# guoyihonggyh/MOBODY-Model-Based-Off-Dynamics-Offline-Reinforcement-Learning

Hardware: AMD Instinct MI355X
Metric: transitions/sec (minibatch rows through train(), refresh amortised at 1/5000) + grad-steps/sec (higher is better)
Workload: dtype f16x2

## Files before the change

### mobody-model-based-off-dynamics-offline-reinforcement-learning_amd/csrc/layers.h

```cpp
#pragma once
#include <stdint.h>
#include <stdlib.h>

#include <type_traits>

#include "../../include/mobody_hip.h"
#include "gather.h"
#include "tile.h"

namespace mobody {

template <int ACT, int MT, class Extra, class Between>
__device__ __forceinline__ void wide_layer(float* Xs, const float* __restrict__ W, const float* __restrict__ b, int Kp,
                                           WideRing& ring, Extra&& extra, Between&& between, uint32_t* mask = nullptr,
                                           bool full = false, int mask_groups = 1 << 30) {
  const float bias0 = b[64 * wave_col() + (lane_id() & 31)], bias1 = b[64 * wave_col() + 32 + (lane_id() & 31)];
  f32x16 acc[MT][2];
  wide_zero<MT>(acc);
  wide_gemm<MT>(Xs, W, Kp, acc, ring);
  if (Kp == HID) TR(3);
  between();
  lds_barrier();
  if (full) {
    wide_foreach<MT>(acc, [&](int row, int col, float v) {
// ... 82 lines not shown
  const unsigned short* w2_planes;
  long long planes_ms;
  float* save_d1;
  float* save_d2;
  unsigned short* save_h1p;
  long long h1p_ms;
  long long h1p_plane;
  int* save_e1;
  int out_mode;
  const float* resid;
  int resid_ld;
  float max_action;
};

constexpr long long DYN_PLANE_MEMBER = 3LL * HID * HID;
__host__ __device__ inline long long dyn_planes_off(int layer, int member) { return ((long long)layer * NENS + member) * DYN_PLANE_MEMBER; }

inline Mlp3FwdArgs fwd_net(const float* blob, const MobodyMlpLayout& L, long long rows) {
  Mlp3FwdArgs a{};
  a.w1 = blob + L.w1; a.b1 = blob + L.b1; a.w2 = blob + L.w2; a.b2 = blob + L.b2; a.w3 = blob + L.w3; a.b3 = blob + L.b3;
  a.sw1 = a.sb1 = a.sw2 = a.sb2 = a.sw3 = a.sb3 = L.member_floats;
  a.Kp1 = L.Kp1; a.Np3 = L.Np3; a.nout = L.out_dim; a.rows = rows;
  return a;
}
inline void fwd_set_planes(Mlp3FwdArgs& a, const float* blob_T, const MobodyMlpLayout& L) {
  a.w2_planes = reinterpret_cast<const unsigned short*>(blob_T + L.w2p);
  a.planes_ms = 2 * L.t_member_floats;
}
inline Mlp3FwdArgs fwd_reward_head(const float* dyn_blob, const MobodyDynLayout& L, const float* dyn_planes, long long rows) {
  Mlp3FwdArgs a{};
  const MobodyLayer &l1 = L.layer[MOBODY_DL_RW1], &l2 = L.layer[MOBODY_DL_RW2], &l3 = L.layer[MOBODY_DL_RW3];
  a.w1 = dyn_blob + l1.w_off; a.b1 = dyn_blob + l1.b_off; a.sw1 = (long long)l1.Kp * l1.Np; a.sb1 = l1.Np;
  a.w2 = dyn_blob + l2.w_off; a.b2 = dyn_blob + l2.b_off; a.sw2 = (long long)l2.Kp * l2.Np; a.sb2 = l2.Np;
  a.w3 = dyn_blob + l3.w_off; a.b3 = dyn_blob + l3.b_off; a.sw3 = (long long)l3.Kp * l3.Np; a.sb3 = l3.Np;
  a.Kp1 = l1.Kp; a.Np3 = l3.Np; a.nout = 1; a.rows = rows;
  if (dyn_planes != nullptr) {
    a.w2_planes = reinterpret_cast<const unsigned short*>(dyn_planes) + dyn_planes_off(2, 0);
    a.planes_ms = DYN_PLANE_MEMBER;
  }
  return a;
}
inline void fwd_set_src(Mlp3FwdArgs& a, int k, const float* src, int ld, int n, long long ms = 0) {
  a.src[k] = src; a.ld[k] = ld; a.n[k] = n; a.src_ms[k] = ms;
}
inline void fwd_set_out(Mlp3FwdArgs& a, float* out, int out_mode, float max_action, const float* resid = nullptr, int resid_ld = 0) {
  a.out = out; a.out_mstride = a.rows * a.nout; a.out_ld = a.nout;
  a.out_mode = out_mode; a.max_action = max_action; a.resid = resid; a.resid_ld = resid_ld;
}
inline void fwd_set_saves(Mlp3FwdArgs& a, float* x, long long x_ms, float* h1, int* e1, float* h2, uint32_t* m1 = nullptr,
                          uint32_t* m2 = nullptr, float* d1 = nullptr, float* d2 = nullptr) {
  if (e1 != nullptr && h1 != nullptr) {
    const long long r32 = (a.rows + 31) & ~31LL;
    a.save_h1p = reinterpret_cast<unsigned short*>(h1); a.h1p_plane = r32 * HID; a.h1p_ms = 2 * r32 * HID; a.save_e1 = e1;
    h1 = nullptr;
  }
  a.save_x = x; a.x_ms = x_ms; a.save_h1 = h1; a.save_h2 = h2; a.mask1 = m1; a.mask2 = m2; a.save_d1 = d1; a.save_d2 = d2;
}

struct FwdGather {
  GatherArgs g;
  int off[2], n[2];
};
inline void fwd_set_gather(FwdGather& fg, int k, const Mlp3FwdArgs& a, int off) {
  fg.off[k] = off; fg.n[k] = a.n[0] + a.n[1] + a.n[2];
}
constexpr int FWD_GATHER_NQ = 2;

template <class F>
inline int dispatch_out_width(int Np3, F&& f) {
  return Np3 == 16 ? f(std::integral_constant<int, 1>{}) : Np3 == 32 ? f(std::integral_constant<int, 2>{})
                                                                     : f(std::integral_constant<int, 0>{});
}

int launch_mlp3_forward(const Mlp3FwdArgs& a, int members_a, const Mlp3FwdArgs& b, int members_b, int act, int prec, hipStream_t st);
inline int launch_mlp3_forward(const Mlp3FwdArgs& a, int members, int act, int prec, hipStream_t st) {
  return launch_mlp3_forward(a, members, Mlp3FwdArgs{}, 0, act, prec, st);
}

int launch_mlp3_forward_gather(const Mlp3FwdArgs& a, int members_a, const Mlp3FwdArgs& b, int members_b, const FwdGather& fg,
                               int prec, hipStream_t st);
int launch_mlp3_fwd_bf_gather(const Mlp3FwdArgs& a, int members_a, const Mlp3FwdArgs& b, int members_b, const FwdGather& fg,
                              int prec, hipStream_t st);

constexpr int MLP_TILE_ROWS = 32;
constexpr int MLP_MT = MLP_TILE_ROWS / 32;

__device__ __forceinline__ int fwd_load_sources(const Mlp3FwdArgs& a, int m, float* Xs, long long row0, int rows_here) {
  int c0 = 0;
#pragma unroll
  for (int k = 0; k < 3; ++k) {
    if (a.n[k] > 0) {
      tile_load(Xs, c0, a.src[k] + m * a.src_ms[k] + row0 * a.ld[k], a.ld[k], a.n[k], 0, rows_here, MLP_TILE_ROWS);
      c0 += a.n[k];
    }
  }
  return c0;
}

template <int NQ>
__device__ __forceinline__ void fwd_gather_rows(const FwdGather& fg, bool second, float* Xs, long long row0, int rows_here) {
  const GatherArgs& g = fg.g;
  const int lane = threadIdx.x & 15, grp = threadIdx.x >> 4;
  const long long N = g.start[g.nbuf];
  const float* mine = nullptr;
  if (lane < 2) {
    const long long r = min(row0 + 16 * lane + grp, N - 1);
    int k;
    const long long src = gather_src(g, r, k);
    mine = g.bufs[k].state + src * g.bufs[k].pitch;
  }
  const int off = second ? fg.off[1] : fg.off[0], n = second ? fg.n[1] : fg.n[0];
  const int q0 = off >> 2, q1 = (off + n + (second ? 2 : 0) + 3) >> 2;
  v4f v[2][NQ];
#pragma unroll
  for (int p = 0; p < 2; ++p) {
    const gather_ptr_t rp = gather_group_row(mine, p);
#pragma unroll
    for (int j = 0; j < NQ; ++j) v[p][j] = rp[min(q0 + lane + 16 * j, q1 - 1)];
  }
#pragma unroll
  for (int p = 0; p < 2; ++p) {
    const int r = 16 * p + grp;
    const bool ok = r < rows_here;
#pragma unroll
    for (int j = 0; j < NQ; ++j) {
      const int q = q0 + lane + 16 * j;
      if (q >= q1) continue;
#pragma unroll
      for (int e = 0; e < 4; ++e) {
        const int c = 4 * q + e - off;
        if (c >= 0 && c < n) Xs[r * LDX + c] = ok ? v[p][j][e] : 0.f;
        if (second && ok && c == n) g.reward[row0 + r] = v[p][j][e];
        if (second && ok && c == n + 1) g.not_done[row0 + r] = v[p][j][e];
      }
    }
  }
}

__device__ __forceinline__ int fwd_gather_tile(const FwdGather& fg, bool second, float* Xs, long long row0, int rows_here) {
  if (blockIdx.x == 0 && blockIdx.y == 0 && threadIdx.x == 0)
    for (int k = 0; k < fg.g.nbump; ++k) fg.g.bump[k][0] += 1;
  const int off = second ? fg.off[1] : fg.off[0], n = second ? fg.n[1] : fg.n[0];
  if (((off + n + (second ? 2 : 0) + 3) >> 2) - (off >> 2) <= 16) fwd_gather_rows<1>(fg, second, Xs, row0, rows_here);
  else fwd_gather_rows<FWD_GATHER_NQ>(fg, second, Xs, row0, rows_here);
  return n;
}

__device__ __forceinline__ void fwd_gather_save(const FwdGather& fg, bool second, int m, const float* Xs, long long row0, int rows_here) {
  const GatherArgs& g = fg.g;
  auto put = [&](float* out, int col0, int n) {
    const uint32_t magic = div_magic(n);
    for (int e = threadIdx.x; e < rows_here * n; e += NTHREADS) {
      const int r = fast_div(e, magic, n);
      out[row0 * n + e] = Xs[r * LDX + col0 + (e - r * n)];
    }
  };
  if (second) {
    put(g.next_state, 0, g.S);
  } else if (m == 0) {
    put(g.state, 0, g.S);
    put(g.action, g.S, g.A);
  }
}

__device__ __forceinline__ void fwd_save_x(const Mlp3FwdArgs& a, int m, const float* Xs, long long row0, int rows_here) {
  if (a.save_x != nullptr && (m == 0 || a.x_ms != 0)) {
    const int c = threadIdx.x & 31, r0 = threadIdx.x >> 5;
    float* sx = a.save_x + m * a.x_ms;
    for (int col = c; col < a.Kp1; col += 32)
      for (int r = r0; r < rows_here; r += NTHREADS >> 5) sx[(row0 + r) * a.Kp1 + col] = Xs[r * LDX + col];
  }
}

struct FwdTileOut { float *h1, *h2; uint32_t *mask1, *mask2; float* out; };
__device__ __forceinline__ FwdTileOut fwd_tile_out(const Mlp3FwdArgs& a, int m, long long row0) {
  FwdTileOut t;
  t.h1 = a.save_h1 ? a.save_h1 + ((long long)m * a.rows + row0) * HID : nullptr;
  t.h2 = a.save_h2 ? a.save_h2 + ((long long)m * a.rows + row0) * HID : nullptr;
  const long long mtile = ((long long)m * ((a.rows + 31) / 32) + row0 / 32) * HID;
  t.mask1 = a.mask1 ? a.mask1 + mtile : nullptr;
  t.mask2 = a.mask2 ? a.mask2 + mtile : nullptr;
  t.out = a.out + m * a.out_mstride + row0 * a.out_ld;
  return t;
}

__device__ __forceinline__ void fwd_emit(const Mlp3FwdArgs& a, float* out, long long row0, int rows_here, int row, int col,
                                         float v, float bias) {
  if (row < rows_here && col < a.nout) {
    float y = v + bias;
    if (a.out_mode == 1) y = a.max_action * tanhf(y);
    if (a.resid != nullptr) y += a.resid[(row0 + row) * a.resid_ld + col];
    out[row * a.out_ld + col] = y;
  }
}

}
```

### mobody-model-based-off-dynamics-offline-reinforcement-learning_amd/csrc/mlp_fwd.hip

```cpp
#include <stdlib.h>

#include "common.h"
#include "layers.h"

namespace mobody {

constexpr int TB = MLP_TILE_ROWS;

template <int ACT, int NT>
__device__ __forceinline__ void mlp3_fwd_tail(const Mlp3FwdArgs& a, int m, float* Xs, WideRing& ring, float* h2,
                                              uint32_t* mask2, float* out, long long row0, int rows_here) {
  const float* w3 = a.w3 + m * a.sw3;
  const float* b3 = a.b3 + m * a.sb3;
  const bool full = rows_here == TB;
  auto save_h2 = [=](auto guarded, int row, int col, float y) {
    if (h2 != nullptr && (!decltype(guarded)::value || row < rows_here)) h2[row * HID + col] = y;
  };
  auto emit = [&](int row, int col, float v, float bias) { fwd_emit(a, out, row0, rows_here, row, col, v, bias); };
  if constexpr (NT > 0) {
    NarrowRegs<NT> br;
    const int mycol = threadIdx.x % (16 * NT);
    float bias;
    wide_layer<ACT, MLP_MT>(Xs, a.w2 + m * a.sw2, a.b2 + m * a.sb2, HID, ring, save_h2, [&] {
      narrow_prefetch<NT>(w3, 16 * NT, br);
// ... 82 lines not shown
  if (!once) {
    int rc = allow_big_lds(k_mlp3_fwd2<ACT_RELU, NT>, 160 * 1024);
    if (rc) return rc;
    once = true;
  }
  const long long rows = a.rows > b.rows ? a.rows : b.rows;
  dim3 grid((unsigned)cdiv(rows, TB), (unsigned)(members_a + members_b));
  ProfScope prof(PROF_MLP_FWD, stream);
  hipLaunchKernelGGL((k_mlp3_fwd2<ACT_RELU, NT>), grid, dim3(NTHREADS), lds, stream, a, b, members_a);
  MB_LAUNCH_OK("k_mlp3_fwd2");
  return 0;
}

static int launch_fwd2_gather(const Mlp3FwdArgs& a, int members_a, const Mlp3FwdArgs& b, int members_b, const FwdGather& fg, hipStream_t stream) {
  size_t lds = (size_t)TB * LDX * sizeof(float);
  static bool once = false;
  if (!once) {
    int rc = allow_big_lds(k_mlp3_fwd2_gather<1>, 160 * 1024);
    if (rc) return rc;
    once = true;
  }
  dim3 grid((unsigned)cdiv(a.rows, TB), (unsigned)(members_a + members_b));
  ProfScope prof(PROF_MLP_FWD, stream);
  hipLaunchKernelGGL(k_mlp3_fwd2_gather<1>, grid, dim3(NTHREADS), lds, stream, a, b, members_a, fg);
  MB_LAUNCH_OK("k_mlp3_fwd2_gather");
  return 0;
}

static int launch_fwd_pair(const Mlp3FwdArgs& a, int members_a, const Mlp3FwdArgs& b, int members_b, hipStream_t stream) {
  return dispatch_out_width(a.Np3, [&](auto nt) { return launch_fwd2_t<decltype(nt)::value>(a, members_a, b, members_b, stream); });
}

template <int ACT>
static int launch_fwd_act(const Mlp3FwdArgs& a, int members, hipStream_t stream) {
  return dispatch_out_width(a.Np3, [&](auto nt) { return launch_fwd_t<ACT, decltype(nt)::value>(a, members, stream); });
}

static int launch_mlp3_fwd(const Mlp3FwdArgs& a, int members, int act, hipStream_t stream) {
  return act == ACT_SWISH ? launch_fwd_act<ACT_SWISH>(a, members, stream) : launch_fwd_act<ACT_RELU>(a, members, stream);
}

int launch_mlp3_fwd_bf(const Mlp3FwdArgs& a, int members_a, const Mlp3FwdArgs& b, int members_b, int act, int prec, hipStream_t st);
int launch_fwd_train(const Mlp3FwdArgs& a, int members, hipStream_t st);

static bool nets_share_launch(const Mlp3FwdArgs& a, const Mlp3FwdArgs& b, int act, int prec) {
  if (act != ACT_RELU) return false;
  return a.Np3 == b.Np3 || (prec == PREC_F16X2 && ((a.Np3 == 16 && b.Np3 == 32) || (a.Np3 == 32 && b.Np3 == 16)));
}

int launch_mlp3_forward(const Mlp3FwdArgs& a, int members_a, const Mlp3FwdArgs& b, int members_b, int act, int prec, hipStream_t st) {
  auto one = [&](const Mlp3FwdArgs& x, int members) {
    if (prec != PREC_F32) return launch_mlp3_fwd_bf(x, members, Mlp3FwdArgs{}, 0, act, prec, st);
    return x.save_d1 != nullptr ? launch_fwd_train(x, members, st) : launch_mlp3_fwd(x, members, act, st);
  };
  const bool has_a = members_a > 0 && a.rows > 0, has_b = members_b > 0 && b.rows > 0;
  if (!has_a || !has_b) return has_a ? one(a, members_a) : has_b ? one(b, members_b) : 0;
  if (!nets_share_launch(a, b, act, prec)) {
    int rc = one(a, members_a);
    return rc ? rc : one(b, members_b);
  }
  return prec == PREC_F32 ? launch_fwd_pair(a, members_a, b, members_b, st) : launch_mlp3_fwd_bf(a, members_a, b, members_b, act, prec, st);
}

int launch_mlp3_forward_gather(const Mlp3FwdArgs& a, int members_a, const Mlp3FwdArgs& b, int members_b, const FwdGather& fg,
                               int prec, hipStream_t st) {
  const GatherArgs& g = fg.g;
  const long long N = g.start[g.nbuf];
  if (N <= 0 || members_a <= 0 || members_b <= 0) return fail(MOBODY_E_ARG, "launch_mlp3_forward_gather: needs both nets and a non-empty minibatch");
  if (a.rows != N || b.rows != N) return fail(MOBODY_E_ARG, "launch_mlp3_forward_gather: the nets run on %lld / %lld rows, the minibatch has %lld", a.rows, b.rows, N);
  for (int k = 0; k < g.nbuf; ++k)
    if (!g.packed[k] && g.start[k + 1] > g.start[k]) return fail(MOBODY_E_ARG, "launch_mlp3_forward_gather: source %d is not a packed ring", k);
  if (fg.off[0] != 0 || fg.n[0] != g.S + g.A || fg.off[1] != g.S + g.A || fg.n[1] != g.S)
    return fail(MOBODY_E_ARG, "launch_mlp3_forward_gather: net a reads state | action, net b next_state");
  auto chunks = [](int off, int n) { return ((off + n + 3) >> 2) - (off >> 2); };
  const bool built = a.Np3 == 16 && (b.Np3 == 16 || (prec == PREC_F16X2 && b.Np3 == 32)) && nets_share_launch(a, b, ACT_RELU, prec) &&
                     chunks(fg.off[0], fg.n[0]) <= 16 * FWD_GATHER_NQ && chunks(fg.off[1], fg.n[1] + 2) <= 16 * FWD_GATHER_NQ;
  if (!built) {
    int rc = launch_gather(g, N, st);
    return rc ? rc : launch_mlp3_forward(a, members_a, b, members_b, ACT_RELU, prec, st);
  }
  return prec == PREC_F32 ? launch_fwd2_gather(a, members_a, b, members_b, fg, st) : launch_mlp3_fwd_bf_gather(a, members_a, b, members_b, fg, prec, st);
}

}

using namespace mobody;

extern "C" int mobody_mlp3_forward(const float* blob, const float* blob_T, int precision, int in_dim, int out_dim,
                                   int members, const float* src0, int n0, const float* src1, int n1, int64_t rows,
                                   int out_mode, float max_action, float* out, float* save_x, float* save_h1,
                                   float* save_h2, void* stream) {
  MobodyMlpLayout L;
  int rc = mobody_mlp_layout(in_dim, out_dim, members, &L);
  if (rc) return rc;
  MB_REQUIRE(rows >= 0, "mobody_mlp3_forward: rows < 0");
  if (rows == 0) return 0;
  MB_REQUIRE(blob && src0 && out, "mobody_mlp3_forward: null pointer");
  MB_REQUIRE(n0 + n1 == in_dim && n0 > 0 && n1 >= 0 && (n1 == 0 || src1), "mobody_mlp3_forward: n0+n1=%d != in_dim=%d", n0 + n1, in_dim);
  rc = check_precision("mobody_mlp3_forward", precision, blob_T != nullptr);
  if (rc) return rc;
  Mlp3FwdArgs a = fwd_net(blob, L, rows);
  fwd_set_src(a, 0, src0, n0, n0);
  fwd_set_src(a, 1, src1, n1, n1);
  fwd_set_out(a, out, out_mode, max_action);
  fwd_set_saves(a, save_x, 0, save_h1, nullptr, save_h2);
  if (precision != PREC_F32) fwd_set_planes(a, blob_T, L);
  return launch_mlp3_forward(a, members, ACT_RELU, precision, as_stream(stream));
}
```

### mobody-model-based-off-dynamics-offline-reinforcement-learning_amd/csrc/mlp_fwd_bf.hip

```cpp
#include <stdlib.h>

#include "common.h"
#include "layers_bf.h"

namespace mobody {

constexpr int TB = MLP_TILE_ROWS, MT = MLP_MT;
constexpr int FWD_L1_RING = 3;
constexpr int FWD_F16_WAVES = 4;

template <int ACT, int PM, int NT, bool DS = false, bool GATHER = false>
__device__ __forceinline__ void mlp3_fwd_bf_tile(const Mlp3FwdArgs& a, int m, float* Xs, const FwdGather* fg = nullptr, bool second = false) {
  char* Ps = reinterpret_cast<char*>(Xs);
  float* scr = reinterpret_cast<float*>(Ps + split_scr_offset<PM, TB>());
  const long long row0 = (long long)blockIdx.x * TB;
  const int rows_here = (int)min((long long)TB, a.rows - row0);
  const bool full = rows_here == TB;
  const float* w1 = a.w1 + m * a.sw1;
  const s16x8* w2b = reinterpret_cast<const s16x8*>(a.w2_planes + m * a.planes_ms);
  const float* w3 = a.w3 + m * a.sw3;
  const float* b3 = a.b3 + m * a.sb3;
  TR(0);
  WideRingT<FWD_L1_RING> ring;
  wide_prefetch(w1, a.Kp1, ring);
  int c0;
  if constexpr (GATHER) {
    c0 = fwd_gather_tile(*fg, second, Xs, row0, rows_here);
  } else if (a.n[0] <= 32 && a.n[1] <= 32 && a.n[2] == 0) {
    tile_load2<TB>(Xs, a.src[0] + m * a.src_ms[0] + row0 * a.ld[0], a.ld[0], a.n[0],
                   a.n[1] > 0 ? a.src[1] + m * a.src_ms[1] + row0 * a.ld[1] : nullptr, a.ld[1], a.n[1], rows_here);
    c0 = a.n[0] + a.n[1];
  } else {
    c0 = fwd_load_sources(a, m, Xs, row0, rows_here);
  }
  tile_zero_cols(Xs, c0, a.Kp1, TB);
  lds_barrier();
  TR(1);
  fwd_save_x(a, m, Xs, row0, rows_here);
  if constexpr (GATHER) fwd_gather_save(*fg, second, m, Xs, row0, rows_here);
  const FwdTileOut t = fwd_tile_out(a, m, row0);
  float* d1 = DS ? a.save_d1 + ((long long)m * a.rows + row0) * HID : nullptr;
  float* d2 = DS ? a.save_d2 + ((long long)m * a.rows + row0) * HID : nullptr;
  const int mg = (rows_here + 31) / 32;
  BfRing<PM> bring;
  PlaneSave gs{nullptr, 0, nullptr};
  if (a.save_h1p != nullptr) {
    gs.base = reinterpret_cast<short*>(a.save_h1p) + m * a.h1p_ms + (row0 / 8) * (HID * 8);
    gs.plane_stride = a.h1p_plane;
    gs.e_out = a.save_e1 + (long long)m * cdiv(a.rows, 32) + row0 / 32;
  }
  const int e1 = wide_layer_to_planes<ACT, MT, PM, TB, DS>(Xs, Ps, scr, w1, a.b1 + m * a.sb1, a.Kp1, ring,
                                                           [&] { bf_prefetch<PM>(w2b, bring); }, t.mask1, full, mg, rows_here, t.h1, gs, d1);
  TR(2);
  auto emit = [&](int row, int col, float v, float bias) { fwd_emit(a, t.out, row0, rows_here, row, col, v, bias); };
  if constexpr (NT > 0) {
    NarrowRegs<NT> br;
    const int mycol = threadIdx.x % (16 * NT);
    float bias;
    bf_layer<ACT, MT, PM, TB, DS>(Xs, Ps, e1, w2b, a.b2 + m * a.sb2, bring, [&] {
      narrow_prefetch<NT>(w3, 16 * NT, br);
      bias = b3[mycol < a.nout ? mycol : 0];
    }, t.mask2, mg, rows_here, t.h2, d2);
    TR(4);
    narrow_run<TB / 16, NT>(Xs, br, [&](int row, int col, float v) { emit(row, col, v, bias); });
  } else {
    bf_layer<ACT, MT, PM, TB, DS>(Xs, Ps, e1, w2b, a.b2 + m * a.sb2, bring, [] {}, t.mask2, mg, rows_here, t.h2, d2);
    narrow_layer(Xs, w3, HID, a.Np3, [&](int row, int col, float v) { emit(row, col, v, b3[col < a.nout ? col : 0]); }, TB);
  }
  TR(5);
}

template <int ACT, int PM, int NT, bool DS = false, int NT2 = NT>
__global__ __launch_bounds__(NTHREADS, (PM == 4 && !DS) ? FWD_F16_WAVES : 2) void k_mlp3_fwd_bf(Mlp3FwdArgs a, Mlp3FwdArgs b, int members_a) {
  extern __shared__ __attribute__((aligned(16))) float Xs[];
  const bool second = (int)blockIdx.y >= members_a;
  const Mlp3FwdArgs s = second ? b : a;
  if ((long long)blockIdx.x * TB >= s.rows) return;
  if constexpr (NT2 == NT) {
    mlp3_fwd_bf_tile<ACT, PM, NT, DS>(s, second ? (int)blockIdx.y - members_a : (int)blockIdx.y, Xs);
  } else {
    if (second) mlp3_fwd_bf_tile<ACT, PM, NT2, DS>(s, (int)blockIdx.y - members_a, Xs);
    else mlp3_fwd_bf_tile<ACT, PM, NT, DS>(s, (int)blockIdx.y, Xs);
  }
}

template <int PM, int NT, int NT2 = NT>
__global__ __launch_bounds__(NTHREADS, PM == 4 ? FWD_F16_WAVES : 2) void k_mlp3_fwd_bf_gather(Mlp3FwdArgs a, Mlp3FwdArgs b, int members_a, FwdGather fg) {
  extern __shared__ __attribute__((aligned(16))) float Xs[];
  const bool second = (int)blockIdx.y >= members_a;
  const Mlp3FwdArgs s = second ? b : a;
  if ((long long)blockIdx.x * TB >= s.rows) return;
  if constexpr (NT2 == NT) {
    mlp3_fwd_bf_tile<ACT_RELU, PM, NT, false, true>(s, second ? (int)blockIdx.y - members_a : (int)blockIdx.y, Xs, &fg, second);
  } else {
    if (second) mlp3_fwd_bf_tile<ACT_RELU, PM, NT2, false, true>(s, (int)blockIdx.y - members_a, Xs, &fg, true);
    else mlp3_fwd_bf_tile<ACT_RELU, PM, NT, false, true>(s, (int)blockIdx.y, Xs, &fg, false);
  }
}

template <int PM, int NT, int NT2 = NT>
static int launch_bf_gather_t(const Mlp3FwdArgs& a, int members_a, const Mlp3FwdArgs& b, int members_b, const FwdGather& fg, hipStream_t st) {
  constexpr size_t lds = split_lds_bytes<PM, TB>();
  static bool once = false;
  if (!once) {
    int rc = allow_big_lds(k_mlp3_fwd_bf_gather<PM, NT, NT2>, 160 * 1024);
    if (rc) return rc;
    once = true;
  }
  ProfScope prof(PROF_MLP_FWD, st);
  hipLaunchKernelGGL((k_mlp3_fwd_bf_gather<PM, NT, NT2>), dim3((unsigned)cdiv(a.rows, TB), (unsigned)(members_a + members_b)),
                     dim3(NTHREADS), lds, st, a, b, members_a, fg);
  MB_LAUNCH_OK("k_mlp3_fwd_bf_gather");
  return 0;
}

int launch_mlp3_fwd_bf_gather(const Mlp3FwdArgs& a, int members_a, const Mlp3FwdArgs& b, int members_b, const FwdGather& fg,
                              int prec, hipStream_t st) {
  if (prec == PREC_F16X2 && b.Np3 == 32) return launch_bf_gather_t<4, 1, 2>(a, members_a, b, members_b, fg, st);
  switch (prec) {
    case PREC_BF16: return launch_bf_gather_t<1, 1>(a, members_a, b, members_b, fg, st);
    case PREC_BF16X2: return launch_bf_gather_t<2, 1>(a, members_a, b, members_b, fg, st);
    case PREC_BF16X3: return launch_bf_gather_t<3, 1>(a, members_a, b, members_b, fg, st);
    default: return launch_bf_gather_t<4, 1>(a, members_a, b, members_b, fg, st);
  }
}

template <int ACT, int PM, int NT, bool DS = false, int NT2 = NT>
static int launch_bf_t(const Mlp3FwdArgs& a, int members_a, const Mlp3FwdArgs& b, int members_b, hipStream_t st) {
  constexpr size_t lds = split_lds_bytes<PM, TB>();
  static bool once = false;
  if (!once) {
    int rc = allow_big_lds(k_mlp3_fwd_bf<ACT, PM, NT, DS, NT2>, 160 * 1024);
    if (rc) return rc;
    once = true;
  }
  const long long rows = a.rows > b.rows ? a.rows : b.rows;
  ProfScope prof(PROF_MLP_FWD, st);
  hipLaunchKernelGGL((k_mlp3_fwd_bf<ACT, PM, NT, DS, NT2>), dim3((unsigned)cdiv(rows, TB), (unsigned)(members_a + members_b)),
                     dim3(NTHREADS), lds, st, a, b, members_a);
  MB_LAUNCH_OK("k_mlp3_fwd_bf");
  return 0;
}

template <int ACT, int PM>
static int launch_bf_nt(const Mlp3FwdArgs& a, int ma, const Mlp3FwdArgs& b, int mb, hipStream_t st) {
  if constexpr (PM == 4 && ACT == ACT_RELU) {
    if (mb > 0 && a.Np3 != b.Np3)
      return a.Np3 == 16 ? launch_bf_t<ACT, PM, 1, false, 2>(a, ma, b, mb, st) : launch_bf_t<ACT, PM, 2, false, 1>(a, ma, b, mb, st);
  }
  return dispatch_out_width(a.Np3, [&](auto nt) { return launch_bf_t<ACT, PM, decltype(nt)::value>(a, ma, b, mb, st); });
}

int launch_mlp3_fwd_bf(const Mlp3FwdArgs& a, int members_a, const Mlp3FwdArgs& b, int members_b, int act, int prec, hipStream_t st) {
// ... 13 lines not shown
```

### mobody-model-based-off-dynamics-offline-reinforcement-learning_amd/csrc/train.hip

```cpp
#include <math.h>

#include "common.h"
#include "layers.h"
#include "train.h"

namespace mobody {

struct TrainWs {
  uint32_t *mq1, *mq2, *ma1, *ma2;
  int *eh1q, *eh1a, *edz2;
  float *pin;
  float *pi, *qt, *q, *qb, *xq, *h1q, *h2q, *xa, *h1a, *h2a, *dz3q, *dz2, *dz1, *dz3a, *dxa, *bcw, *dbp, *slabs, *lossp;
  float *bc;
  int *tickets;
  long long total;
  int nsplit_q, nsplit_a, ntiles;
  MobodyMlpLayout Lq, La;
};

static int carve(const MobodyTrainDims& d, float* base, TrainWs& w) {
  int rc = mobody_mlp_layout(d.S + d.A, 1, 2, &w.Lq);
  if (rc) return rc;
  rc = mobody_mlp_layout(d.S, d.A, 1, &w.La);
  if (rc) return rc;
// ... 158 lines not shown
                            long long rows, float* out, int out_mode, float max_action, float* sx, float* sh1,
                            float* sh2, uint32_t* m1 = nullptr, uint32_t* m2 = nullptr, const float* blob_T = nullptr,
                            int* e1 = nullptr) {
  Mlp3FwdArgs a = fwd_net(blob, L, rows);
  if (blob_T != nullptr) fwd_set_planes(a, blob_T, L);
  fwd_set_src(a, 0, s0, n0, n0);
  fwd_set_src(a, 1, s1, n1, s1 ? n1 : 0);
  fwd_set_out(a, out, out_mode, max_action);
  fwd_set_saves(a, sx, 0, sh1, e1, sh2, m1, m2);
  return a;
}

static int weight_grads(const MobodyMlpLayout& L, const float* x, const float* h1, const float* h2, const int* e_h1, const float* dz3,
                        long long rows, const TrainWs& w, float* grad, const LossFinal& loss, const AdamTarget& adam, int prec,
                        hipStream_t st) {
  const bool actor = L.members == 1;
  Mlp3WgradArgs g = wgrad_net(L, rows, actor ? w.nsplit_a : w.nsplit_q);
  wgrad_set_saves(g, x, 0, h1, h2, e_h1);
  wgrad_set_grads(g, dz3, w.dz2, w.dz1, w.dbp, w.ntiles, w.edz2);
  wgrad_set_scratch(g, w.slabs, w.bc + (actor ? 2 : 0));
  wgrad_set_result(g, grad, loss, adam, prec);
  return mlp3_weight_grads(g, st);
}

static Mlp3BwdArgs bwd_args(const MobodyMlpLayout& L, const float* blob_T, const float* dz3, const float* h1,
                            const float* h2, long long rows, float* dz2, float* dz1, float* dbp,
                            const uint32_t* m1 = nullptr, const uint32_t* m2 = nullptr, int prec = PREC_F32, int* e2 = nullptr) {
  Mlp3BwdArgs b = bwd_net(L, blob_T, rows);
  bwd_set_planes(b, L, prec);
  bwd_set_acts(b, h1, h2, m1, m2, 0);
  bwd_set_grads(b, dz3, dz2, dz1, dbp, prec == PREC_F16X2 ? e2 : nullptr);
  return b;
}

}

using namespace mobody;

extern "C" int64_t mobody_train_workspace(const MobodyTrainDims* d) {
  if (check_dims(d, "mobody_train_workspace")) return -1;
  TrainWs w;
  if (carve(*d, nullptr, w)) return -1;
  return w.total;
}

static int critic_impl(const MobodyCritic& a, const FwdGather* gather, void* stream) {
  const char* who = "mobody_critic";
  const MobodyTrainDims* d = &a.d;
  const MobodyHyper* h = &a.h;
  const bool fused = a.m != nullptr;
  int rc = check_dims(d, who);
  if (rc) return rc;
  MB_REQUIRE(a.q_blob && a.q_blob_T && a.state && a.action && a.reward && a.not_done && a.loss_out && a.workspace, "%s: null pointer", who);
  MB_REQUIRE(a.q_next || (a.actor_blob && a.qtarg_blob && a.next_state), "%s: need q_next or actor/target/next_state", who);
  rc = check_precision(who, h->precision, a.q_next != nullptr || (a.actor_blob_T && a.qtarg_blob_T));
  if (rc) return rc;
  if (fused) {
    MB_REQUIRE(a.qtarg_blob, "%s: null pointer", who);
    MB_REQUIRE(a.t_dev != nullptr || a.t >= 1, "%s: step t must be >= 1", who);
    MB_REQUIRE(a.bump == nullptr || a.bump != a.t_dev, "%s: bump must not be the step word the launch reads", who);
  } else {
    MB_REQUIRE(a.bump == nullptr, "%s: bump is incremented by the optimizer launch: it needs m, v", who);
  }
  TrainWs w;
  rc = carve(*d, a.workspace, w);
  if (rc) return rc;
  AdamTarget adam{};
  if (fused) {
    adam = adam_target(a.q_blob, a.q_blob_T, a.m, a.v, a.qtarg_blob, a.t, a.t_dev, a.lr, h->tau, 1.f, h->precision);
    adam.target_T = a.qtarg_blob_T;
    adam.bump = (long long*)a.bump;
  }
  const float *q_blob = a.q_blob, *state = a.state, *action = a.action, *next_state = a.next_state, *q_next = a.q_next;
  const int prec = h->precision;
  const float *aT = prec != PREC_F32 ? a.actor_blob_T : nullptr, *qT = prec != PREC_F32 ? a.q_blob_T : nullptr, *tT = prec != PREC_F32 ? a.qtarg_blob_T : nullptr;
  hipStream_t st = as_stream(stream);
  const long long N = d->N;
  const int S = d->S, A = d->A;
  const Mlp3FwdArgs fq = fwd_args(q_blob, w.Lq, state, S, action, A, N, w.q, 0, 1.f, w.xq, w.h1q, w.h2q, w.mq1, w.mq2, qT,
                                  prec == PREC_F16X2 ? w.eh1q : nullptr);
  if (a.phase == 2) {
  } else if (q_next == nullptr) {
    const Mlp3FwdArgs fpn = fwd_args(a.actor_blob, w.La, next_state, S, nullptr, 0, N, w.pin, 1, h->max_action, nullptr, nullptr, nullptr, nullptr, nullptr, aT);
    if (gather != nullptr) {
      FwdGather fg = *gather;
      fwd_set_gather(fg, 0, fq, 0);
      fwd_set_gather(fg, 1, fpn, S + A);
      rc = launch_mlp3_forward_gather(fq, 2, fpn, 1, fg, prec, st);
    } else {
      rc = launch_mlp3_forward(fq, 2, fpn, 1, ACT_RELU, prec, st);
    }
    const Mlp3FwdArgs ft = fwd_args(a.qtarg_blob, w.Lq, next_state, S, w.pin, A, N, w.qt, 0, 1.f, nullptr, nullptr, nullptr, nullptr, nullptr, tT);
    if (!rc && a.policy_forward)
      rc = launch_mlp3_forward(ft, 2, fwd_args(a.actor_blob, w.La, state, S, nullptr, 0, N, w.pi, 1, h->max_action, w.xa, w.h1a, w.h2a, w.ma1, w.ma2, aT,
                                               prec == PREC_F16X2 ? w.eh1a : nullptr), 1, ACT_RELU, prec, st);
    else if (!rc)
      rc = launch_mlp3_forward(ft, 2, ACT_RELU, prec, st);
  } else {
    rc = launch_mlp3_forward(fq, 2, ACT_RELU, prec, st);
  }
  if (rc || a.phase == 1) return rc;
  const float invNg = 1.f / (float)d->N_global;
  Mlp3BwdArgs bq = bwd_args(w.Lq, a.q_blob_T, w.dz3q, w.h1q, w.h2q, N, w.dz2, w.dz1, w.dbp, w.mq1, w.mq2, prec, w.edz2);
  bq.seed.mode = 1; bq.seed.q = w.q; bq.seed.qt = w.qt; bq.seed.qnext = q_next; bq.seed.r = a.reward; bq.seed.nd = a.not_done;
  bq.seed.gamma = h->gamma; bq.seed.inv_ng = invNg; bq.seed.dz3_out = w.dz3q; bq.seed.lossp = w.lossp;
  rc = launch_mlp3_bwd(bq, 2, false, st);
  if (rc) return rc;
  LossFinal lf{};
  lf.kind = 1; lf.nparts = 2 * w.ntiles; lf.scale = invNg; lf.parts = w.lossp; lf.out = a.loss_out;
  return weight_grads(w.Lq, w.xq, w.h1q, w.h2q, w.eh1q, w.dz3q, N, w, a.grad_q, lf, adam, prec, st);
}

extern "C" int mobody_critic(const MobodyCritic* a, void* stream) {
  const char* who = "mobody_critic";
  MB_BLOCK(who, a, MobodyCritic);
  MB_REQUIRE((a->grad_q != nullptr) != (a->m != nullptr || a->v != nullptr), "%s: exactly one of grad_q and the optimizer state m, v must be given", who);
  MB_REQUIRE(a->grad_q || (a->m && a->v), "%s: null pointer", who);
  MB_REQUIRE(a->phase >= 0 && a->phase <= 2, "%s: phase is 0 (the whole step), 1 (forwards) or 2 (backward + update)", who);
  if (a->gather == nullptr) return critic_impl(*a, nullptr, stream);
  const MobodyGatherRng* gr = a->gather;
  MB_REQUIRE(a->phase == 0, "%s: the step cannot be split (phase %d): the first forward launch writes the minibatch the backward reads", who, a->phase);
  MB_REQUIRE(a->q_next == nullptr, "%s: q_next given: the launch that gathers is the one that evaluates pi(s')", who);
  FwdGather fg{};
  long long N;
  int rc = gather_args_rng(who, fg.g, gr->bufs, gr->counts, gr->nbuf, a->d.S, a->d.A, gr->seeds, gr->call_offsets, gr->counter, gr->sizes,
                           a->state, a->action, a->next_state, a->reward, a->not_done, gr->bump, gr->nbump, N);
  if (rc) return rc;
  MB_REQUIRE(N == a->d.N, "%s: the counts add up to %lld rows, the step runs on %lld", who, N, (long long)a->d.N);
  for (int k = 0; k < gr->nbuf; ++k)
    MB_REQUIRE(gr->counts[k] == 0 || fg.g.packed[k], "%s: source %d is not a row-interleaved ring (mobody_ring_pitch)", who, k);
  return critic_impl(*a, &fg, stream);
}

extern "C" int mobody_actor_forward(const MobodyActor* a, void* stream) {
  const char* who = "mobody_actor_forward";
  MB_BLOCK(who, a, MobodyActor);
  const MobodyTrainDims* d = &a->d;
  const MobodyHyper* h = &a->h;
  int rc = check_dims(d, who);
  if (rc) return rc;
  MB_REQUIRE(a->actor_blob && a->q_blob && a->state && a->action && a->stats && a->workspace, "%s: null pointer", who);
  rc = check_precision(who, h->precision, a->actor_blob_T && a->q_blob_T);
  if (rc) return rc;
  const int prec = h->precision;
  const float *aT = prec != PREC_F32 ? a->actor_blob_T : nullptr, *qT = prec != PREC_F32 ? a->q_blob_T : nullptr;
  const float *q_blob = a->q_blob, *state = a->state;
  TrainWs w;
  rc = carve(*d, a->workspace, w);
  if (rc) return rc;
  hipStream_t st = as_stream(stream);
  const long long N = d->N, Nt = d->Nt;
  const int S = d->S, A = d->A;
  const Mlp3FwdArgs fb = fwd_args(q_blob, w.Lq, state, S, a->action, A, Nt, w.qb, 0, 1.f, nullptr, nullptr, nullptr, nullptr, nullptr, qT);
  const Mlp3FwdArgs fp = fwd_args(q_blob, w.Lq, state, S, w.pi, A, N, w.q, 0, 1.f, nullptr, nullptr, nullptr, w.mq1, w.mq2, qT);
  if (a->policy_ready) {
    rc = launch_mlp3_forward(fb, 2, fp, 2, ACT_RELU, prec, st);
  } else {
    rc = launch_mlp3_forward(fb, 2, fwd_args(a->actor_blob, w.La, state, S, nullptr, 0, N, w.pi, 1, h->max_action, w.xa, w.h1a, w.h2a, w.ma1, w.ma2, aT,
                                             prec == PREC_F16X2 ? w.eh1a : nullptr), 1, ACT_RELU, prec, st);
    if (!rc) rc = launch_mlp3_forward(fp, 2, ACT_RELU, prec, st);
  }
  if (rc) return rc;
  hipLaunchKernelGGL(k_actor_stats, dim3(1), dim3(1024), 0, st, w.q, w.qb, N, Nt, a->stats, w.tickets, w.ntiles);
  MB_LAUNCH_OK("k_actor_stats");
  return 0;
}

static int actor_backward_impl(const MobodyActor& a, void* stream) {
  const char* who = "mobody_actor_backward";
  const MobodyTrainDims* d = &a.d;
  const MobodyHyper* h = &a.h;
  const bool fused = a.m != nullptr;
  int rc = check_dims(d, who);
  if (rc) return rc;
  MB_REQUIRE(a.actor_blob && a.actor_blob_T && a.q_blob && a.q_blob_T && a.state && a.action && a.stats && a.loss_out && a.workspace,
             "%s: null pointer", who);
  rc = check_precision(who, h->precision, true);
  if (rc) return rc;
  MB_REQUIRE(!fused || a.t_dev != nullptr || a.t >= 1, "%s: step t must be >= 1", who);
  TrainWs w;
// ... 103 lines not shown
```

Before: 50.07 million.

## Fuse critic forward passes into one kernel chaining next-action into target Q via LDS

Merges the gathered critic forward (Q, next-state actor) and the target-Q/policy forward into a single launch. Workgroups are split by role along blockIdx.y, and the actor-on-next-state tile passes its output action to the target-Q tile through shared memory instead of a global round trip and a second launch. For small batches the target-Q members run as two chains, otherwise one chain does both members serially. The change removes a kernel launch and a global dependency, but it makes the chained workgroups longer, uses more LDS, and falls back to the old path when its eligibility conditions are not met.

```diff
diff --git a/mobody-model-based-off-dynamics-offline-reinforcement-learning_amd/csrc/critic_fwd_bf.hip b/mobody-model-based-off-dynamics-offline-reinforcement-learning_amd/csrc/critic_fwd_bf.hip
--- /dev/null
+++ b/mobody-model-based-off-dynamics-offline-reinforcement-learning_amd/csrc/critic_fwd_bf.hip
@@ -0,0 +1,66 @@
+#include <stdlib.h>
+
+#include "fwd_bf_tile.h"
+
+namespace mobody {
+
+__device__ __forceinline__ bool opaque_true() {
+  int one;
+  asm volatile("s_mov_b32 %0, 1" : "=s"(one));
+  return one != 0;
+}
+
+template <int PM, int NT2, int CHAINS>
+__global__ __launch_bounds__(NTHREADS, PM == 4 ? FWD_F16_WAVES : 2) void k_critic_fwd_bf(Mlp3FwdArgs q, Mlp3FwdArgs pn, Mlp3FwdArgs qt, Mlp3FwdArgs pi,
+                                                                                         FwdGather fg) {
+  extern __shared__ __attribute__((aligned(16))) float Xs[];
+  const int role = (int)blockIdx.y;
+  CriticFwdTile ch;
+  ch.Sa = Xs + split_lds_bytes<PM, TB>() / sizeof(float);
+  ch.S = fg.g.S; ch.A = fg.g.A;
+  ch.chained = role < CHAINS; ch.owes = role == 0;
+  if (role < CHAINS) {
+    if (opaque_true()) mlp3_fwd_bf_tile<ACT_RELU, PM, NT2, false, true, CF_NEXT>(pn, 0, Xs, &fg, true, ch);
+    if constexpr (CHAINS == 1) {
+      if (opaque_true()) mlp3_fwd_bf_tile<ACT_RELU, PM, 1, false, true, CF_Q>(qt, 0, Xs, &fg, false, ch);
+      if (opaque_true()) mlp3_fwd_bf_tile<ACT_RELU, PM, 1, false, true, CF_Q>(qt, 1, Xs, &fg, false, ch);
+    } else {
+      if (opaque_true()) mlp3_fwd_bf_tile<ACT_RELU, PM, 1, false, true, CF_Q>(qt, role, Xs, &fg, false, ch);
+    }
+  } else if (role < CHAINS + 2) {
+    mlp3_fwd_bf_tile<ACT_RELU, PM, 1, false, true, CF_Q>(q, role - CHAINS, Xs, &fg, false, ch);
+  } else {
+    mlp3_fwd_bf_tile<ACT_RELU, PM, NT2, false, true, CF_PI>(pi, 0, Xs, &fg, false, ch);
+  }
+}
+
+size_t critic_fwd_bf_lds(int S, int A) { return split_lds_bytes<4, TB>() + (size_t)TB * (S + A) * sizeof(float); }
+
+template <int NT2, int CHAINS>
+static int launch_critic_fwd_bf_t(const Mlp3FwdArgs& q, const Mlp3FwdArgs& pn, const Mlp3FwdArgs& qt, const Mlp3FwdArgs* pi, const FwdGather& fg,
+                                  hipStream_t st) {
+  static bool once = false;
+  if (!once) {
+    int rc = allow_big_lds(k_critic_fwd_bf<4, NT2, CHAINS>, 160 * 1024);
+    if (rc) return rc;
+    once = true;
+  }
+  ProfScope prof(PROF_MLP_FWD, st);
+  hipLaunchKernelGGL((k_critic_fwd_bf<4, NT2, CHAINS>), dim3((unsigned)cdiv(q.rows, TB), (unsigned)(CHAINS + 2 + (pi != nullptr ? 1 : 0))),
+                     dim3(NTHREADS), critic_fwd_bf_lds(fg.g.S, fg.g.A), st, q, pn, qt, pi != nullptr ? *pi : Mlp3FwdArgs{}, fg);
+  MB_LAUNCH_OK("k_critic_fwd_bf");
+  return 0;
+}
+
+#ifndef MOBODY_CRITIC_FWD_TWO_CHAIN_WGS
+#define MOBODY_CRITIC_FWD_TWO_CHAIN_WGS 512
+#endif
+
+int launch_critic_fwd_bf(const Mlp3FwdArgs& q, const Mlp3FwdArgs& pn, const Mlp3FwdArgs& qt, const Mlp3FwdArgs* pi, const FwdGather& fg,
+                         hipStream_t st) {
+  const bool two = 5 * cdiv(q.rows, TB) <= MOBODY_CRITIC_FWD_TWO_CHAIN_WGS;
+  if (pn.Np3 == 32) return two ? launch_critic_fwd_bf_t<2, 2>(q, pn, qt, pi, fg, st) : launch_critic_fwd_bf_t<2, 1>(q, pn, qt, pi, fg, st);
+  return two ? launch_critic_fwd_bf_t<1, 2>(q, pn, qt, pi, fg, st) : launch_critic_fwd_bf_t<1, 1>(q, pn, qt, pi, fg, st);
+}
+
+}
diff --git a/mobody-model-based-off-dynamics-offline-reinforcement-learning_amd/csrc/fwd_bf_tile.h b/mobody-model-based-off-dynamics-offline-reinforcement-learning_amd/csrc/fwd_bf_tile.h
--- /dev/null
+++ b/mobody-model-based-off-dynamics-offline-reinforcement-learning_amd/csrc/fwd_bf_tile.h
@@ -0,0 +1,127 @@
+#pragma once
+#include "common.h"
+#include "layers_bf.h"
+
+namespace mobody {
+
+constexpr int TB = MLP_TILE_ROWS, MT = MLP_MT;
+constexpr int FWD_L1_RING = 3;
+constexpr int FWD_F16_WAVES = 4;
+
+enum CriticFwdRole { CF_NONE = 0, CF_NEXT = 1, CF_Q = 2, CF_PI = 3 };
+struct CriticFwdTile {
+  float* Sa;
+  int S, A;
+  bool chained;
+  bool owes;
+};
+
+__device__ __forceinline__ void chain_emit(const Mlp3FwdArgs& a, float* out, int rows_here, int row, int col, float v, float bias,
+                                           const CriticFwdTile& ch) {
+  if (col >= a.nout) return;
+  float y = 0.f;
+  if (row < rows_here) {
+    y = v + bias;
+    if (a.out_mode == 1) y = a.max_action * tanhf(y);
+    if (ch.owes) out[row * a.out_ld + col] = y;
+  }
+  ch.Sa[row * (ch.S + ch.A) + ch.S + col] = y;
+}
+__device__ __forceinline__ void chain_stash(const float* Xs, const CriticFwdTile& ch) {
+  const int c = threadIdx.x & 31, r0 = threadIdx.x >> 5;
+  for (int col = c; col < ch.S; col += 32)
+#pragma unroll
+    for (int u = 0; u < TB / 8; ++u) ch.Sa[(r0 + 8 * u) * (ch.S + ch.A) + col] = Xs[(r0 + 8 * u) * LDX + col];
+}
+__device__ __forceinline__ int chain_input(float* Xs, const CriticFwdTile& ch) {
+  const int c = threadIdx.x & 31, r0 = threadIdx.x >> 5;
+  for (int col = c; col < ch.S + ch.A; col += 32)
+#pragma unroll
+    for (int u = 0; u < TB / 8; ++u) Xs[(r0 + 8 * u) * LDX + col] = ch.Sa[(r0 + 8 * u) * (ch.S + ch.A) + col];
+  return ch.S + ch.A;
+}
+
+template <int ACT, int PM, int NT, bool DS = false, bool GATHER = false, int ROLE = CF_NONE>
+__device__ __forceinline__ void mlp3_fwd_bf_tile(const Mlp3FwdArgs& a, int m, float* Xs, const FwdGather* fg = nullptr, bool second = false,
+                                                 const CriticFwdTile& ch = CriticFwdTile{}) {
+  char* Ps = reinterpret_cast<char*>(Xs);
+  float* scr = reinterpret_cast<float*>(Ps + split_scr_offset<PM, TB>());
+  const long long row0 = (long long)blockIdx.x * TB;
+  const int rows_here = (int)min((long long)TB, a.rows - row0);
+  const bool full = rows_here == TB;
+  const float* w1 = a.w1 + m * a.sw1;
+  const s16x8* w2b = reinterpret_cast<const s16x8*>(a.w2_planes + m * a.planes_ms);
+  const float* w3 = a.w3 + m * a.sw3;
+  const float* b3 = a.b3 + m * a.sb3;
+  TR(0);
+  WideRingT<FWD_L1_RING> ring;
+  wide_prefetch(w1, a.Kp1, ring);
+  int c0;
+  if constexpr (ROLE == CF_NEXT) {
+    c0 = fwd_gather_tile(*fg, true, Xs, row0, rows_here, ch.owes);
+  } else if constexpr (ROLE == CF_Q) {
+    if (ch.chained) {
+      lds_barrier();
+      c0 = chain_input(Xs, ch);
+    } else {
+      c0 = fwd_gather_tile(*fg, false, Xs, row0, rows_here);
+    }
+  } else if constexpr (ROLE == CF_PI) {
+    c0 = fwd_gather_tile<FWD_COLS_STATE>(*fg, false, Xs, row0, rows_here);
+  } else if constexpr (GATHER) {
+    c0 = fwd_gather_tile(*fg, second, Xs, row0, rows_here);
+  } else if (a.n[0] <= 32 && a.n[1] <= 32 && a.n[2] == 0) {
+    tile_load2<TB>(Xs, a.src[0] + m * a.src_ms[0] + row0 * a.ld[0], a.ld[0], a.n[0],
+                   a.n[1] > 0 ? a.src[1] + m * a.src_ms[1] + row0 * a.ld[1] : nullptr, a.ld[1], a.n[1], rows_here);
+    c0 = a.n[0] + a.n[1];
+  } else {
+    c0 = fwd_load_sources(a, m, Xs, row0, rows_here);
+  }
+  tile_zero_cols(Xs, c0, a.Kp1, TB);
+  lds_barrier();
+  TR(1);
+  fwd_save_x(a, m, Xs, row0, rows_here);
+  if constexpr (ROLE == CF_NEXT) {
+    if (ch.owes) fwd_gather_save(*fg, true, m, Xs, row0, rows_here);
+    chain_stash(Xs, ch);
+  } else if constexpr (ROLE == CF_Q) {
+    if (!ch.chained) fwd_gather_save(*fg, false, m, Xs, row0, rows_here);
+  } else if constexpr (ROLE == CF_NONE && GATHER) {
+    fwd_gather_save(*fg, second, m, Xs, row0, rows_here);
+  }
+  const FwdTileOut t = fwd_tile_out(a, m, row0);
+  float* d1 = DS ? a.save_d1 + ((long long)m * a.rows + row0) * HID : nullptr;
+  float* d2 = DS ? a.save_d2 + ((long long)m * a.rows + row0) * HID : nullptr;
+  const int mg = (rows_here + 31) / 32;
+  BfRing<PM> bring;
+  PlaneSave gs{nullptr, 0, nullptr};
+  if (a.save_h1p != nullptr) {
+    gs.base = reinterpret_cast<short*>(a.save_h1p) + m * a.h1p_ms + (row0 / 8) * (HID * 8);
+    gs.plane_stride = a.h1p_plane;
+    gs.e_out = a.save_e1 + (long long)m * cdiv(a.rows, 32) + row0 / 32;
+  }
+  const int e1 = wide_layer_to_planes<ACT, MT, PM, TB, DS>(Xs, Ps, scr, w1, a.b1 + m * a.sb1, a.Kp1, ring,
+                                                           [&] { bf_prefetch<PM>(w2b, bring); }, t.mask1, full, mg, rows_here, t.h1, gs, d1);
+  TR(2);
+  auto emit = [&](int row, int col, float v, float bias) {
+    if constexpr (ROLE == CF_NEXT) chain_emit(a, t.out, rows_here, row, col, v, bias, ch);
+    else fwd_emit(a, t.out, row0, rows_here, row, col, v, bias);
+  };
+  if constexpr (NT > 0) {
+    NarrowRegs<NT> br;
+    const int mycol = threadIdx.x % (16 * NT);
+    float bias;
+    bf_layer<ACT, MT, PM, TB, DS>(Xs, Ps, e1, w2b, a.b2 + m * a.sb2, bring, [&] {
+      narrow_prefetch<NT>(w3, 16 * NT, br);
+      bias = b3[mycol < a.nout ? mycol : 0];
+    }, t.mask2, mg, rows_here, t.h2, d2);
+    TR(4);
+    narrow_run<TB / 16, NT>(Xs, br, [&](int row, int col, float v) { emit(row, col, v, bias); });
+  } else {
+    bf_layer<ACT, MT, PM, TB, DS>(Xs, Ps, e1, w2b, a.b2 + m * a.sb2, bring, [] {}, t.mask2, mg, rows_here, t.h2, d2);
+    narrow_layer(Xs, w3, HID, a.Np3, [&](int row, int col, float v) { emit(row, col, v, b3[col < a.nout ? col : 0]); }, TB);
+  }
+  TR(5);
+}
+
+}
diff --git a/mobody-model-based-off-dynamics-offline-reinforcement-learning_amd/csrc/layers.h b/mobody-model-based-off-dynamics-offline-reinforcement-learning_amd/csrc/layers.h
--- a/mobody-model-based-off-dynamics-offline-reinforcement-learning_amd/csrc/layers.h
+++ b/mobody-model-based-off-dynamics-offline-reinforcement-learning_amd/csrc/layers.h
@@ -188,6 +188,13 @@
 int launch_mlp3_fwd_bf_gather(const Mlp3FwdArgs& a, int members_a, const Mlp3FwdArgs& b, int members_b, const FwdGather& fg,
                               int prec, hipStream_t st);
 
+int launch_critic_forward_gather(const Mlp3FwdArgs& q, const Mlp3FwdArgs& pn, const Mlp3FwdArgs& qt, const Mlp3FwdArgs* pi,
+                                 const FwdGather& fg, int prec, hipStream_t st);
+int launch_critic_fwd_bf(const Mlp3FwdArgs& q, const Mlp3FwdArgs& pn, const Mlp3FwdArgs& qt, const Mlp3FwdArgs* pi, const FwdGather& fg,
+                         hipStream_t st);
+size_t critic_fwd_bf_lds(int S, int A);
+constexpr size_t CRITIC_FWD_LDS_MAX = 40 * 1024;
+
 constexpr int MLP_TILE_ROWS = 32;
 constexpr int MLP_MT = MLP_TILE_ROWS / 32;
 
@@ -203,8 +210,9 @@
   return c0;
 }
 
-template <int NQ>
-__device__ __forceinline__ void fwd_gather_rows(const FwdGather& fg, bool second, float* Xs, long long row0, int rows_here) {
+enum FwdGatherCols { FWD_COLS_NET = 0, FWD_COLS_STATE = 1 };
+template <int NQ, int COLS = FWD_COLS_NET>
+__device__ __forceinline__ void fwd_gather_rows(const FwdGather& fg, bool second, float* Xs, long long row0, int rows_here, bool owes = true) {
   const GatherArgs& g = fg.g;
   const int lane = threadIdx.x & 15, grp = threadIdx.x >> 4;
   const long long N = g.start[g.nbuf];
@@ -215,7 +223,7 @@
     const long long src = gather_src(g, r, k);
     mine = g.bufs[k].state + src * g.bufs[k].pitch;
   }
-  const int off = second ? fg.off[1] : fg.off[0], n = second ? fg.n[1] : fg.n[0];
+  const int off = second ? fg.off[1] : fg.off[0], n = COLS == FWD_COLS_STATE ? g.S : second ? fg.n[1] : fg.n[0];
   const int q0 = off >> 2, q1 = (off + n + (second ? 2 : 0) + 3) >> 2;
   v4f v[2][NQ];
 #pragma unroll
@@ -236,19 +244,20 @@
       for (int e = 0; e < 4; ++e) {
         const int c = 4 * q + e - off;
         if (c >= 0 && c < n) Xs[r * LDX + c] = ok ? v[p][j][e] : 0.f;
-        if (second && ok && c == n) g.reward[row0 + r] = v[p][j][e];
-        if (second && ok && c == n + 1) g.not_done[row0 + r] = v[p][j][e];
+        if (second && ok && owes && c == n) g.reward[row0 + r] = v[p][j][e];
+        if (second && ok && owes && c == n + 1) g.not_done[row0 + r] = v[p][j][e];
       }
     }
   }
 }
 
-__device__ __forceinline__ int fwd_gather_tile(const FwdGather& fg, bool second, float* Xs, long long row0, int rows_here) {
+template <int COLS = FWD_COLS_NET>
+__device__ __forceinline__ int fwd_gather_tile(const FwdGather& fg, bool second, float* Xs, long long row0, int rows_here, bool owes = true) {
   if (blockIdx.x == 0 && blockIdx.y == 0 && threadIdx.x == 0)
     for (int k = 0; k < fg.g.nbump; ++k) fg.g.bump[k][0] += 1;
-  const int off = second ? fg.off[1] : fg.off[0], n = second ? fg.n[1] : fg.n[0];
-  if (((off + n + (second ? 2 : 0) + 3) >> 2) - (off >> 2) <= 16) fwd_gather_rows<1>(fg, second, Xs, row0, rows_here);
-  else fwd_gather_rows<FWD_GATHER_NQ>(fg, second, Xs, row0, rows_here);
+  const int off = second ? fg.off[1] : fg.off[0], n = COLS == FWD_COLS_STATE ? fg.g.S : second ? fg.n[1] : fg.n[0];
+  if (((off + n + (second ? 2 : 0) + 3) >> 2) - (off >> 2) <= 16) fwd_gather_rows<1, COLS>(fg, second, Xs, row0, rows_here, owes);
+  else fwd_gather_rows<FWD_GATHER_NQ, COLS>(fg, second, Xs, row0, rows_here, owes);
   return n;
 }
 
diff --git a/mobody-model-based-off-dynamics-offline-reinforcement-learning_amd/csrc/mlp_fwd.hip b/mobody-model-based-off-dynamics-offline-reinforcement-learning_amd/csrc/mlp_fwd.hip
--- a/mobody-model-based-off-dynamics-offline-reinforcement-learning_amd/csrc/mlp_fwd.hip
+++ b/mobody-model-based-off-dynamics-offline-reinforcement-learning_amd/csrc/mlp_fwd.hip
@@ -188,6 +188,37 @@
   return prec == PREC_F32 ? launch_fwd2_gather(a, members_a, b, members_b, fg, st) : launch_mlp3_fwd_bf_gather(a, members_a, b, members_b, fg, prec, st);
 }
 
+static bool critic_forward_merges(const Mlp3FwdArgs& q, const Mlp3FwdArgs& pn, const Mlp3FwdArgs& qt, const Mlp3FwdArgs* pi, const FwdGather& fg,
+                                  int prec) {
+#ifdef MOBODY_TWO_CRITIC_FWD
+  return false;
+#else
+  const GatherArgs& g = fg.g;
+  const long long N = g.start[g.nbuf];
+  auto chunks = [](int off, int n) { return ((off + n + 3) >> 2) - (off >> 2); };
+  if (prec != PREC_F16X2 || N <= 0 || q.rows != N || pn.rows != N || qt.rows != N || (pi != nullptr && pi->rows != N)) return false;
+  for (int k = 0; k < g.nbuf; ++k)
+    if (!g.packed[k] && g.start[k + 1] > g.start[k]) return false;
+  if (fg.off[0] != 0 || fg.n[0] != g.S + g.A || fg.off[1] != g.S + g.A || fg.n[1] != g.S) return false;
+  if (q.Np3 != 16 || qt.Np3 != 16 || (pn.Np3 != 16 && pn.Np3 != 32) || chunks(0, g.S + g.A) > 16 * FWD_GATHER_NQ ||
+      chunks(g.S + g.A, g.S + 2) > 16 * FWD_GATHER_NQ)
+    return false;
+  if (qt.Kp1 != q.Kp1 || qt.n[0] != g.S || qt.n[1] != g.A || qt.n[2] != 0 || qt.src[1] != pn.out || pn.nout != g.A ||
+      pn.out_ld != g.A || pn.resid != nullptr || qt.save_x || qt.save_h1 || qt.save_h1p || qt.save_h2 || qt.mask1 || qt.mask2)
+    return false;
+  if (pi != nullptr && (pi->Np3 != pn.Np3 || pi->Kp1 != pn.Kp1 || pi->n[0] != g.S || pi->n[1] + pi->n[2] != 0)) return false;
+  return critic_fwd_bf_lds(g.S, g.A) <= CRITIC_FWD_LDS_MAX;
+#endif
+}
+
+int launch_critic_forward_gather(const Mlp3FwdArgs& q, const Mlp3FwdArgs& pn, const Mlp3FwdArgs& qt, const Mlp3FwdArgs* pi,
+                                 const FwdGather& fg, int prec, hipStream_t st) {
+  if (critic_forward_merges(q, pn, qt, pi, fg, prec)) return launch_critic_fwd_bf(q, pn, qt, pi, fg, st);
+  int rc = launch_mlp3_forward_gather(q, 2, pn, 1, fg, prec, st);
+  if (rc) return rc;
+  return pi != nullptr ? launch_mlp3_forward(qt, 2, *pi, 1, ACT_RELU, prec, st) : launch_mlp3_forward(qt, 2, ACT_RELU, prec, st);
+}
+
 }
 
 using namespace mobody;
diff --git a/mobody-model-based-off-dynamics-offline-reinforcement-learning_amd/csrc/mlp_fwd_bf.hip b/mobody-model-based-off-dynamics-offline-reinforcement-learning_amd/csrc/mlp_fwd_bf.hip
--- a/mobody-model-based-off-dynamics-offline-reinforcement-learning_amd/csrc/mlp_fwd_bf.hip
+++ b/mobody-model-based-off-dynamics-offline-reinforcement-learning_amd/csrc/mlp_fwd_bf.hip
@@ -1,74 +1,8 @@
 #include <stdlib.h>
 
-#include "common.h"
-#include "layers_bf.h"
+#include "fwd_bf_tile.h"
 
 namespace mobody {
-
-constexpr int TB = MLP_TILE_ROWS, MT = MLP_MT;
-constexpr int FWD_L1_RING = 3;
-constexpr int FWD_F16_WAVES = 4;
-
-template <int ACT, int PM, int NT, bool DS = false, bool GATHER = false>
-__device__ __forceinline__ void mlp3_fwd_bf_tile(const Mlp3FwdArgs& a, int m, float* Xs, const FwdGather* fg = nullptr, bool second = false) {
-  char* Ps = reinterpret_cast<char*>(Xs);
-  float* scr = reinterpret_cast<float*>(Ps + split_scr_offset<PM, TB>());
-  const long long row0 = (long long)blockIdx.x * TB;
-  const int rows_here = (int)min((long long)TB, a.rows - row0);
-  const bool full = rows_here == TB;
-  const float* w1 = a.w1 + m * a.sw1;
-  const s16x8* w2b = reinterpret_cast<const s16x8*>(a.w2_planes + m * a.planes_ms);
-  const float* w3 = a.w3 + m * a.sw3;
-  const float* b3 = a.b3 + m * a.sb3;
-  TR(0);
-  WideRingT<FWD_L1_RING> ring;
-  wide_prefetch(w1, a.Kp1, ring);
-  int c0;
-  if constexpr (GATHER) {
-    c0 = fwd_gather_tile(*fg, second, Xs, row0, rows_here);
-  } else if (a.n[0] <= 32 && a.n[1] <= 32 && a.n[2] == 0) {
-    tile_load2<TB>(Xs, a.src[0] + m * a.src_ms[0] + row0 * a.ld[0], a.ld[0], a.n[0],
-                   a.n[1] > 0 ? a.src[1] + m * a.src_ms[1] + row0 * a.ld[1] : nullptr, a.ld[1], a.n[1], rows_here);
-    c0 = a.n[0] + a.n[1];
-  } else {
-    c0 = fwd_load_sources(a, m, Xs, row0, rows_here);
-  }
-  tile_zero_cols(Xs, c0, a.Kp1, TB);
-  lds_barrier();
-  TR(1);
-  fwd_save_x(a, m, Xs, row0, rows_here);
-  if constexpr (GATHER) fwd_gather_save(*fg, second, m, Xs, row0, rows_here);
-  const FwdTileOut t = fwd_tile_out(a, m, row0);
-  float* d1 = DS ? a.save_d1 + ((long long)m * a.rows + row0) * HID : nullptr;
-  float* d2 = DS ? a.save_d2 + ((long long)m * a.rows + row0) * HID : nullptr;
-  const int mg = (rows_here + 31) / 32;
-  BfRing<PM> bring;
-  PlaneSave gs{nullptr, 0, nullptr};
-  if (a.save_h1p != nullptr) {
-    gs.base = reinterpret_cast<short*>(a.save_h1p) + m * a.h1p_ms + (row0 / 8) * (HID * 8);
-    gs.plane_stride = a.h1p_plane;
-    gs.e_out = a.save_e1 + (long long)m * cdiv(a.rows, 32) + row0 / 32;
-  }
-  const int e1 = wide_layer_to_planes<ACT, MT, PM, TB, DS>(Xs, Ps, scr, w1, a.b1 + m * a.sb1, a.Kp1, ring,
-                                                           [&] { bf_prefetch<PM>(w2b, bring); }, t.mask1, full, mg, rows_here, t.h1, gs, d1);
-  TR(2);
-  auto emit = [&](int row, int col, float v, float bias) { fwd_emit(a, t.out, row0, rows_here, row, col, v, bias); };
-  if constexpr (NT > 0) {
-    NarrowRegs<NT> br;
-    const int mycol = threadIdx.x % (16 * NT);
-    float bias;
-    bf_layer<ACT, MT, PM, TB, DS>(Xs, Ps, e1, w2b, a.b2 + m * a.sb2, bring, [&] {
-      narrow_prefetch<NT>(w3, 16 * NT, br);
-      bias = b3[mycol < a.nout ? mycol : 0];
-    }, t.mask2, mg, rows_here, t.h2, d2);
-    TR(4);
-    narrow_run<TB / 16, NT>(Xs, br, [&](int row, int col, float v) { emit(row, col, v, bias); });
-  } else {
-    bf_layer<ACT, MT, PM, TB, DS>(Xs, Ps, e1, w2b, a.b2 + m * a.sb2, bring, [] {}, t.mask2, mg, rows_here, t.h2, d2);
-    narrow_layer(Xs, w3, HID, a.Np3, [&](int row, int col, float v) { emit(row, col, v, b3[col < a.nout ? col : 0]); }, TB);
-  }
-  TR(5);
-}
 
 template <int ACT, int PM, int NT, bool DS = false, int NT2 = NT>
 __global__ __launch_bounds__(NTHREADS, (PM == 4 && !DS) ? FWD_F16_WAVES : 2) void k_mlp3_fwd_bf(Mlp3FwdArgs a, Mlp3FwdArgs b, int members_a) {
diff --git a/mobody-model-based-off-dynamics-offline-reinforcement-learning_amd/csrc/train.hip b/mobody-model-based-off-dynamics-offline-reinforcement-learning_amd/csrc/train.hip
--- a/mobody-model-based-off-dynamics-offline-reinforcement-learning_amd/csrc/train.hip
+++ b/mobody-model-based-off-dynamics-offline-reinforcement-learning_amd/csrc/train.hip
@@ -264,20 +264,21 @@
   if (a.phase == 2) {
   } else if (q_next == nullptr) {
     const Mlp3FwdArgs fpn = fwd_args(a.actor_blob, w.La, next_state, S, nullptr, 0, N, w.pin, 1, h->max_action, nullptr, nullptr, nullptr, nullptr, nullptr, aT);
+    const Mlp3FwdArgs ft = fwd_args(a.qtarg_blob, w.Lq, next_state, S, w.pin, A, N, w.qt, 0, 1.f, nullptr, nullptr, nullptr, nullptr, nullptr, tT);
+    Mlp3FwdArgs fpi{};
+    if (a.policy_forward)
+      fpi = fwd_args(a.actor_blob, w.La, state, S, nullptr, 0, N, w.pi, 1, h->max_action, w.xa, w.h1a, w.h2a, w.ma1, w.ma2, aT,
+                     prec == PREC_F16X2 ? w.eh1a : nullptr);
     if (gather != nullptr) {
       FwdGather fg = *gather;
       fwd_set_gather(fg, 0, fq, 0);
       fwd_set_gather(fg, 1, fpn, S + A);
-      rc = launch_mlp3_forward_gather(fq, 2, fpn, 1, fg, prec, st);
+      rc = launch_critic_forward_gather(fq, fpn, ft, a.policy_forward ? &fpi : nullptr, fg, prec, st);
     } else {
       rc = launch_mlp3_forward(fq, 2, fpn, 1, ACT_RELU, prec, st);
+      if (!rc && a.policy_forward) rc = launch_mlp3_forward(ft, 2, fpi, 1, ACT_RELU, prec, st);
+      else if (!rc) rc = launch_mlp3_forward(ft, 2, ACT_RELU, prec, st);
     }
-    const Mlp3FwdArgs ft = fwd_args(a.qtarg_blob, w.Lq, next_state, S, w.pin, A, N, w.qt, 0, 1.f, nullptr, nullptr, nullptr, nullptr, nullptr, tT);
-    if (!rc && a.policy_forward)
-      rc = launch_mlp3_forward(ft, 2, fwd_args(a.actor_blob, w.La, state, S, nullptr, 0, N, w.pi, 1, h->max_action, w.xa, w.h1a, w.h2a, w.ma1, w.ma2, aT,
-                                               prec == PREC_F16X2 ? w.eh1a : nullptr), 1, ACT_RELU, prec, st);
-    else if (!rc)
-      rc = launch_mlp3_forward(ft, 2, ACT_RELU, prec, st);
   } else {
     rc = launch_mlp3_forward(fq, 2, ACT_RELU, prec, st);
   }
```

New measurement: 52.97 million (median of 6 runs). 5.8% higher.
